# awentzonline/tartangan

Measured on AMD Instinct MI355X. Metric: images/sec (G+D step), higher is better.
Workload: dtype f32; 1 GPU; 128:3 SA-GAN cnn G+D step (R1 penalty, Adam x2, EMA), 128x128 RGB, batch 64/GPU, global batch 64; trainer=cnn, gan_config=128:3, global_batch=64, parallelism=dp1, hip_graphs=True

## Files before the change

include/tartangan_amd.h:

```cpp
#ifndef TARTANGAN_AMD_H
#define TARTANGAN_AMD_H

#include <stddef.h>
#include <stdint.h>

#ifdef __cplusplus
extern "C" {
#endif

#define TG_OK 0
#define TG_EINVAL (-1)
#define TG_EUNSUPPORTED (-2)
#define TG_EWORKSPACE (-3)

int tg_version(void);
const char* tg_arch(void);

int tg_conv2d_fwd(const float* x, const float* w, const float* bias ,
                  const float* residual ,
                  float* y, int B, int Cin, int Cout, int H, int W, int ks, void* stream);
int tg_conv2d_fwd_up2res(const float* x, const float* w, const float* bias , const float* residual_lo,
                         float* y, int B, int Cin, int Cout, int H, int W, void* stream);
int tg_upconv3x3_weights(const float* w, float* wp, int Cout, int Cin, void* stream);
int tg_upconv3x3_fwd(const float* a, const float* wp, const float* bias , const float* residual ,
                     float* y, int B, int Cin, int Cout, int H, int W, void* stream);
int tg_upconv3x3_weights_t(const float* w, float* w4t, int Cout, int Cin, void* stream);
int tg_upconv3x3_weights_pair(const float* w, float* wp, float* w4t, int Cout, int Cin, void* stream);
int tg_upconv3x3_dgrad_supported(int B, int Cin, int Cout, int H, int W);
int tg_upconv3x3_dgrad(const float* gy, const float* w4t, float* ga, int B, int Cin, int Cout, int H, int W, void* stream);
int tg_poolconv3x3_weights(const float* w, float* w4, float* wp, int Cout, int Cin, void* stream);
int tg_poolconv3x3_supported(int B, int Cin, int Cout, int H, int W);
int tg_poolconv3x3_fwd(const float* x, const float* w4, const float* bias , const float* residual ,
                       float* y, int B, int Cin, int Cout, int H, int W, void* stream);
int tg_poolconv3x3_dgrad(const float* gy, const float* wp, float* gx, int B, int Cin, int Cout, int H, int W, void* stream);
size_t tg_poolconv3x3_wgrad_workspace(int B, int Cin, int Cout, int H, int W);
int tg_poolconv3x3_wgrad(const float* x , const float* gy , float* gw, float* workspace,
                         size_t workspace_bytes, int B, int Cin, int Cout, int H, int W, int accumulate, float* gbias ,
                         void* stream);
size_t tg_upconv3x3_wgrad_workspace(int B, int Cin, int Cout, int H, int W);
int tg_upconv3x3_wgrad(const float* a , const float* gy , float* gw, float* workspace,
                       size_t workspace_bytes, int B, int Cin, int Cout, int H, int W, int accumulate, float* gbias ,
                       void* stream);
int tg_conv2d_dgrad(const float* gy, const float* w, float* gx,
                    int B, int Cin, int Cout, int H, int W, int ks, void* stream);
size_t tg_conv2d_wgrad_workspace(int B, int Cin, int Cout, int H, int W, int ks);
int tg_conv2d_wgrad(const float* x, const float* gy, float* gw, float* gbias ,
                    float* workspace, size_t workspace_bytes,
                    int B, int Cin, int Cout, int H, int W, int ks, int accumulate, void* stream);
int tg_conv1x1_multi_supported(int c0, int c1, int c2, int B, int Cin, int H, int W);
int tg_conv1x1_multi_fwd(const float* x, const float* w, float* y0, float* y1, float* y2, int c0, int c1, int c2,
                         int B, int Cin, int H, int W, void* stream);
int tg_conv1x1_multi_dgrad(const float* gy0, const float* gy1, const float* gy2, const float* w, float* gx,
                           int c0, int c1, int c2, int B, int Cin, int H, int W, void* stream);
size_t tg_conv1x1_multi_wgrad_workspace(int c0, int c1, int c2, int B, int Cin, int H, int W);
int tg_conv1x1_multi_wgrad(const float* x, const float* gy0, const float* gy1, const float* gy2, float* gw,
                           float* workspace, size_t workspace_bytes, int c0, int c1, int c2, int B, int Cin, int H, int W,
                           int accumulate , void* stream);
typedef int64_t tg_host_i64;
#define TG_WGRAD_ITEM_FIELDS 10
int tg_conv2d_wgrad_partials(const float* x, const float* gy, float* workspace, size_t workspace_bytes,
                             int B, int Cin, int Cout, int H, int W, int ks, int want_bias, void* stream);
int tg_conv2d_wgrad_reduce_batch(const tg_host_i64* items , int n_items, void* stream);
#define TG_FORM_ITEM_FIELDS 5
int tg_poolconv3x3_weights_batch(const tg_host_i64* items , int n_items, void* stream);
int tg_rgb_compose_fwd(const float* w1, const float* b1, const float* w3, float* wc, int Cout, int C, int Cimg, void* stream);
int tg_rgb_compose_bwd(const float* gwc, const float* w1, const float* b1, const float* w3, float* gw1, float* gb1, float* gw3, int Cout,
                       int C, int Cimg, int accumulate, void* stream);
int tg_poolconv3x3_wgrad_partials(const float* x, const float* gy, float* workspace, size_t workspace_bytes, int B, int Cin, int Cout,
                                  int H, int W, int want_bias, void* stream);
int tg_upconv3x3_wgrad_partials(const float* a, const float* gy, float* workspace, size_t workspace_bytes, int B, int Cin, int Cout,
                                int H, int W, int want_bias, void* stream);
int tg_s2_wgrad_reduce_batch(const tg_host_i64* items , int n_items, void* stream);
int tg_channel_sum(const float* x, float* out, float* workspace, int B, int C, int HW, int accumulate,
                   void* stream);
int tg_channel_bcast(const float* v, float* out, int B, int C, int HW, void* stream);

int tg_gemm(const float* A, const float* Bm, float* C, const float* bias_n ,
            int M, int N, int K, int lda, int ldb, int ldc, int transA, int transB,
            int batch, int64_t strideA, int64_t strideB, int64_t strideC, float beta, void* stream);

size_t tg_bn_workspace(int B, int C, int HW);
int tg_bn_train_stats(const float* x, float* mean, float* invstd,
                      float* running_mean , float* running_var ,
                      int64_t* num_batches_tracked ,
                      float momentum, float eps, float* workspace, int B, int C, int HW, int replicate, void* stream);
int tg_bn_train_fwd(const float* x, float* mean, float* invstd,
                    float* running_mean , float* running_var ,
                    int64_t* num_batches_tracked , const float* gamma, const float* beta,
                    float slope, float momentum, float eps, float* z, float* workspace,
                    int B, int C, int HW, int replicate, void* stream);
int tg_bn_eval_stats(const float* running_mean, const float* running_var, float* mean, float* invstd,
                     float eps, int C, void* stream);
int tg_bn_act_fwd(const float* x, const float* mean, const float* invstd, const float* gamma,
                  const float* beta, float slope, float* z, int B, int C, int HW, void* stream);
int tg_bn_act_bwd(const float* gz, const float* x, const float* mean, const float* invstd,
                  const float* gamma, const float* beta, float slope, int training,
                  float* gx , float* ggamma, float* gbeta, float* workspace,
                  int B, int C, int HW, int accumulate ,
                  const float* gx_add ,
                  void* stream);
int tg_bn_train_fwd_groups(const float* x, float* mean, float* invstd,
                           float* running_mean , float* running_var ,
                           int64_t* num_batches_tracked , const float* gamma, const float* beta,
                           float slope, float momentum, float eps, float* z, float* workspace,
                           int groups, int B, int C, int HW, int replicate, void* stream);
int tg_bn_act_bwd_groups(const float* gz, const float* x, const float* mean, const float* invstd,
                         const float* gamma, const float* beta, float slope, int training,
                         float* gx , float* ggamma, float* gbeta, float* workspace,
                         int groups, int B, int C, int HW, int accumulate,
                         const float* gx_add , int add_groups, void* stream);
int tg_bn_act_dbwd(const float* v, const float* vgamma , const float* vbeta ,
                   const float* gz, const float* x, const float* mean, const float* invstd,
                   const float* gamma, const float* beta, float slope,
                   float* adj_gz, float* adj_x, float* adj_gamma, float* workspace,
                   int B, int C, int HW, int accumulate , void* stream);

int tg_bn_sync_stats_local(const float* x, double* sums , float* workspace, int B, int C, int HW,
                           void* stream);
int tg_bn_sync_stats_finish(const double* sums , int world, float* mean, float* invstd,
                            float* running_mean , float* running_var ,
                            int64_t* num_batches_tracked , float momentum, float eps,
                            int64_t count_global, int replicate, int C, void* stream);
int tg_bn_sync_bwd_local(const float* gz, const float* x, const float* mean, const float* invstd,
                         const float* gamma, const float* beta, float slope, double* sums ,
                         float* workspace, int B, int C, int HW, void* stream);
int tg_bn_sync_bwd_finish(const float* gz, const float* x, const float* mean, const float* invstd,
                          const float* gamma, const float* beta, float slope,
                          const double* local_sums , const double* global_sums ,
                          int64_t count_global, float* gx , float* ggamma, float* gbeta,
                          float* workspace, int B, int C, int HW, int accumulate,
                          const float* gx_add , void* stream);
int tg_bn_sync_dbwd_local(const float* v, const float* gz, const float* x, const float* mean,
                          const float* invstd, const float* gamma, const float* beta, float slope,
                          double* sums , float* workspace, int B, int C, int HW, void* stream);
int tg_bn_sync_dbwd_finish(const float* v, const float* gz, const float* x, const float* mean,
                           const float* invstd, const float* gamma, const float* beta, float slope,
                           const double* global_sums , int64_t count_global, int world,
                           float* adj_gz, float* adj_x, float* adj_gamma, float* workspace,
                           int B, int C, int HW, int accumulate , void* stream);

int tg_up2x(const float* x, float* y, float alpha, int BC, int H, int W, void* stream);
int tg_pool2(const float* x, const float* residual ,
             float* y, float alpha, int BC, int H, int W, void* stream);
int tg_bilinear_half_fwd(const float* x, float* y, int BC, int H, int W, void* stream);
int tg_bilinear_half_bwd(const float* gy, const float* residual , float* gx,
// ... 149 lines not shown
```

tartangan_amd/csrc/conv.hip:

```cpp
#include <cstdlib>
#include <type_traits>
#include <utility>

#include "common.h"

namespace {

typedef float f32x16 __attribute__((ext_vector_type(16)));
typedef float f32x4 __attribute__((ext_vector_type(4)));

constexpr int CT_THREADS = 256;

template <int TH_, int TW_, int NI_>
struct Geo {
  static constexpr int TH = TH_, TW = TW_, NI = NI_, NPIX = TH_ * TW_ * NI_;
  static_assert(NPIX == 256 || NPIX == 64, "a pixel tile is 256 pixels (waves split pixels) or 64 (waves split K)");
  static constexpr int PPW = (NPIX == 64) ? 64 : NPIX / 4;
  static_assert(TW_ % 4 == 0, "rows are staged as float4");
};
using G4 = Geo<4, 4, 16>;
using G8 = Geo<8, 8, 4>;
using G16 = Geo<16, 16, 1>;
using GX = Geo<8, 32, 1>;
using G4k = Geo<4, 4, 4>;
// ... 1088 lines not shown
      if ((i + 1) * CT_THREADS <= PCHP || i * CT_THREADS + wave * 64 < PCHP) dma16(rx, buf + (i * CT_THREADS + wave * 64) * 4, off);
    }
#pragma unroll
    for (int i = 0; i < NVG; ++i) {
      const int e = i * CT_THREADS + threadIdx.x;
      const int co = e / WGD_GYQ, q = e % WGD_GYQ;
      const int p = 4 * q;
      const int img = p / (G::TH * G::TW), rem = p % (G::TH * G::TW);
      const int hh = tc.h0 + rem / G::TW, ww = tc.w0 + rem % G::TW;
      const bool ok = (e < GCH) && (q < 64) && (co0 + co < s.Cout) && (tc.b0 + img < s.B) && (hh < s.H) && (ww < s.W);
      const uint32_t off = ok ? (__umul24(__umul24(img, s.Cout) + co, HW) + __umul24(hh, s.W) + ww) << 2 : DMA_OOB;
      if ((i + 1) * CT_THREADS <= GCHP || i * CT_THREADS + wave * 64 < GCHP) dma16(rg, buf + PBUF + (i * CT_THREADS + wave * 64) * 4, off);
    }
  };
  auto compute = [&](const float* buf) {
    const float* pl = buf;
    const float* gl = buf + PBUF;
    if (s.prio) __builtin_amdgcn_s_setprio(0);
#pragma unroll
    for (int g = 0; g < 16; ++g) {
      constexpr int PPI = G::TH * G::TW;
      const int pg = 4 * g;
      const int goff = ((pg / PPI) * P::PH + (pg % PPI) / G::TW) * P::PWS + (pg % G::TW);
      float a[MTW], b[NT];
#pragma unroll
      for (int m = 0; m < MTW; ++m) a[m] = gl[lane_a + m * 16 * WG_GYS + 4 * g];
#pragma unroll
      for (int n = 0; n < NT; ++n) b[n] = pl[colbase[n] + lane_b + goff];
#pragma unroll
      for (int m = 0; m < MTW; ++m) bsum[m] += a[m];
#pragma unroll
      for (int m = 0; m < MTW; ++m)
#pragma unroll
        for (int n = 0; n < NT; ++n) acc[m][n] = __builtin_amdgcn_mfma_f32_16x16x4f32(a[m], b[n], acc[m][n], 0, 0, 0);
    }
    if (s.prio) __builtin_amdgcn_s_setprio(3);
  };

  for (int t = split; t < ntiles; t += S) {
    __syncthreads();
    issue(t, lds);
    asm volatile("s_waitcnt vmcnt(0)" ::: "memory");
    __syncthreads();
    compute(lds);
  }

  __syncthreads();
  float* red = lds;
#pragma unroll
  for (int m = 0; m < MTW; ++m)
#pragma unroll
    for (int n = 0; n < NT; ++n)
#pragma unroll
      for (int r = 0; r < 4; ++r) red[(((wave * MTW + m) * NT + n) * 4 + r) * 64 + lane] = acc[m][n][r];
  constexpr int PER_WAVE = MTW * NT * 4 * 64;
  float* bred = lds + 4 * PER_WAVE;
  if (do_bias) {
#pragma unroll
    for (int m = 0; m < MTW; ++m) {
      float v = bsum[m];
      v += __shfl_xor(v, 16, 64);
      v += __shfl_xor(v, 32, 64);
      if (h == 0) bred[wave * CT + m * 16 + j] = v;
    }
  }
  __syncthreads();
  for (int e = threadIdx.x; e < PER_WAVE; e += CT_THREADS) {
    const float v = (red[e] + red[PER_WAVE + e]) + (red[2 * PER_WAVE + e] + red[3 * PER_WAVE + e]);
    const int l = e & 63, q = e >> 6;
    const int r = q & 3, n = (q >> 2) % NT, m = (q >> 2) / NT;
    const int col = n * 16 + (l & 15);
    const int co = co0 + m * 16 + (l >> 4) * 4 + r;
    const int ci = ci0 + col / KK, tap = col % KK;
    if (col < NCOL && co < s.Cout && ci < s.Cin)
      part[(((int64_t)split * s.Cout + co) * s.Cin + ci) * KK + tap] = v;
  }
  if (do_bias && threadIdx.x < CT && co0 + (int)threadIdx.x < s.Cout) {
    const int c = threadIdx.x;
    bias_part[(int64_t)split * s.Cout + co0 + c] = (bred[c] + bred[CT + c]) + (bred[2 * CT + c] + bred[3 * CT + c]);
  }
}

template <int MT, int NT>
__global__ void __launch_bounds__(256)
conv1x1_wgrad_stream_kernel(const float* __restrict__ x, ChanSegs gys, float* __restrict__ part,
                            float* __restrict__ bias_part , int Cin, int Cout, int HW, int64_t groups, int S) {
  __shared__ float red[4 * MT * NT * 4 * 64 + 4 * 16 * MT];
  const int lane = threadIdx.x & 63, wave = threadIdx.x >> 6, j = lane & 15, h = lane >> 4;
  const int co0 = blockIdx.y * 16 * MT, ci0 = blockIdx.z * 16 * NT, split = blockIdx.x;
  const int64_t g_begin = groups * split / S, g_end = groups * (split + 1) / S;
  const int64_t n = g_end - g_begin;
  const int64_t w_begin = g_begin + n * wave / 4, w_end = g_begin + n * (wave + 1) / 4;
  const int gpp = HW >> 4;
  int64_t arow[MT], brow[NT], aimg[MT];
  const float* abase[MT];
#pragma unroll
  for (int m = 0; m < MT; ++m) {
    const int co = min(co0 + 16 * m + j, Cout - 1), k = gys.find(co);
    abase[m] = gys.p[k];
    aimg[m] = (int64_t)gys.width(k) * HW;
    arow[m] = (int64_t)(co - gys.start[k]) * HW + 4 * h;
  }
#pragma unroll
  for (int t = 0; t < NT; ++t) brow[t] = (int64_t)min(ci0 + 16 * t + j, Cin - 1) * HW + 4 * h;
  f32x4 acc[MT][NT];
#pragma unroll
  for (int m = 0; m < MT; ++m)
#pragma unroll
    for (int t = 0; t < NT; ++t) acc[m][t] = f32x4{0.f, 0.f, 0.f, 0.f};
  float bsum[MT];
#pragma unroll
  for (int m = 0; m < MT; ++m) bsum[m] = 0.f;
  constexpr int U = 4;
  for (int64_t g0 = w_begin; g0 < w_end; g0 += U) {
    float4 ga[U][MT], xb[U][NT];
#pragma unroll
    for (int u = 0; u < U; ++u) {
      const int64_t g = g0 + u;
      const bool ok = g < w_end;
      const int64_t b = ok ? g / gpp : 0;
      const int64_t p = ok ? (g - b * gpp) * 16 : 0;
#pragma unroll
      for (int m = 0; m < MT; ++m)
        ga[u][m] = ok ? *reinterpret_cast<const float4*>(abase[m] + b * aimg[m] + arow[m] + p) : make_float4(0.f, 0.f, 0.f, 0.f);
#pragma unroll
      for (int t = 0; t < NT; ++t)
        xb[u][t] = ok ? *reinterpret_cast<const float4*>(x + b * Cin * HW + brow[t] + p) : make_float4(0.f, 0.f, 0.f, 0.f);
    }
#pragma unroll
    for (int u = 0; u < U; ++u) {
#pragma unroll
      for (int m = 0; m < MT; ++m) bsum[m] += (ga[u][m].x + ga[u][m].y) + (ga[u][m].z + ga[u][m].w);
#pragma unroll
      for (int m = 0; m < MT; ++m) {
        const float av[4] = {ga[u][m].x, ga[u][m].y, ga[u][m].z, ga[u][m].w};
#pragma unroll
        for (int t = 0; t < NT; ++t) {
          const float bv[4] = {xb[u][t].x, xb[u][t].y, xb[u][t].z, xb[u][t].w};
#pragma unroll
          for (int r = 0; r < 4; ++r) acc[m][t] = __builtin_amdgcn_mfma_f32_16x16x4f32(av[r], bv[r], acc[m][t], 0, 0, 0);
        }
      }
    }
  }
  constexpr int PER_WAVE = MT * NT * 4 * 64;
#pragma unroll
  for (int m = 0; m < MT; ++m)
#pragma unroll
    for (int t = 0; t < NT; ++t)
#pragma unroll
      for (int i = 0; i < 4; ++i) red[wave * PER_WAVE + ((m * NT + t) * 4 + i) * 64 + lane] = acc[m][t][i];
  float* bred = red + 4 * PER_WAVE;
  const bool do_bias = bias_part != nullptr && blockIdx.z == 0;
  if (do_bias) {
#pragma unroll
    for (int m = 0; m < MT; ++m) {
      float v = bsum[m];
      v += __shfl_xor(v, 16, 64);
      v += __shfl_xor(v, 32, 64);
      if (h == 0) bred[wave * 16 * MT + 16 * m + j] = v;
    }
  }
  __syncthreads();
  for (int e = threadIdx.x; e < PER_WAVE; e += 256) {
    const float v = (red[e] + red[PER_WAVE + e]) + (red[2 * PER_WAVE + e] + red[3 * PER_WAVE + e]);
    const int l = e & 63, q = e >> 6;
    const int i = q & 3, t = (q >> 2) % NT, m = (q >> 2) / NT;
    const int co = co0 + 16 * m + 4 * (l >> 4) + i, ci = ci0 + 16 * t + (l & 15);
    if (co < Cout && ci < Cin) part[((int64_t)split * Cout + co) * Cin + ci] = v;
  }
  if (do_bias && threadIdx.x < 16 * MT && co0 + (int)threadIdx.x < Cout) {
    const int c = threadIdx.x;
    bias_part[(int64_t)split * Cout + co0 + c] = (bred[c] + bred[16 * MT + c]) + (bred[2 * 16 * MT + c] + bred[3 * 16 * MT + c]);
  }
}

static inline bool conv1x1_wgrad_stream_ok(const float* x, const float* gy, const Shape& s) {
  return (s.H * s.W) % 16 == 0 && tg_aligned16(x) && tg_aligned16(gy);
}
static int launch_conv1x1_wgrad_segs(const float* x, ChanSegs gy, float* part, float* bias_part, Shape s, int S, hipStream_t st) {
  const int HW = s.H * s.W;
  const int64_t groups = (int64_t)s.B * (HW / 16);
  const int mt = s.Cout > 16 ? 2 : 1, nt = s.Cin > 16 ? 2 : 1;
  dim3 grid(S, (s.Cout + 16 * mt - 1) / (16 * mt), (s.Cin + 16 * nt - 1) / (16 * nt));
  if (mt == 1 && nt == 1) conv1x1_wgrad_stream_kernel<1, 1><<<grid, 256, 0, st>>>(x, gy, part, bias_part, s.Cin, s.Cout, HW, groups, S);
  else if (mt == 1) conv1x1_wgrad_stream_kernel<1, 2><<<grid, 256, 0, st>>>(x, gy, part, bias_part, s.Cin, s.Cout, HW, groups, S);
  else if (nt == 1) conv1x1_wgrad_stream_kernel<2, 1><<<grid, 256, 0, st>>>(x, gy, part, bias_part, s.Cin, s.Cout, HW, groups, S);
  else conv1x1_wgrad_stream_kernel<2, 2><<<grid, 256, 0, st>>>(x, gy, part, bias_part, s.Cin, s.Cout, HW, groups, S);
  return tg_launch_status();
}
static int launch_conv1x1_wgrad_stream(const float* x, const float* gy, float* part, float* bias_part, Shape s, int S, hipStream_t st) {
  return launch_conv1x1_wgrad_segs(x, one_seg(gy, s.Cout), part, bias_part, s, S, st);
}

__device__ __forceinline__ void wgrad_reduce_block(int blk, const float* __restrict__ part, float* __restrict__ gw, int64_t E, int S,
                                                   const float* __restrict__ bias_part, float* __restrict__ gbias, int Cout,
                                                   int accumulate) {
  __shared__ float red[4][64];
  const int lane = threadIdx.x & 63, wave = threadIdx.x >> 6;
  const int eblocks = (int)((E + 63) / 64);
  const float* src = part;
  float* dst = gw;
  int64_t n = E, e = blk * 64ll + lane;
  if (blk >= eblocks) {
    src = bias_part; dst = gbias; n = Cout;
    e = (blk - eblocks) * 64ll + lane;
  }
  float a0 = 0.f, a1 = 0.f, a2 = 0.f, a3 = 0.f;
  if (e < n) {
    int sidx = wave;
    for (; sidx + 12 < S; sidx += 16) {
      a0 += src[(int64_t)sidx * n + e];
      a1 += src[(int64_t)(sidx + 4) * n + e];
      a2 += src[(int64_t)(sidx + 8) * n + e];
      a3 += src[(int64_t)(sidx + 12) * n + e];
    }
    for (; sidx < S; sidx += 4) a0 += src[(int64_t)sidx * n + e];
  }
  red[wave][lane] = (a0 + a1) + (a2 + a3);
  __syncthreads();
  if (wave == 0 && e < n) {
    const float r = (red[0][lane] + red[1][lane]) + (red[2][lane] + red[3][lane]);
    dst[e] = accumulate ? dst[e] + r : r;
  }
}

__global__ void __launch_bounds__(256) wgrad_reduce_kernel(const float* __restrict__ part, float* __restrict__ gw, int64_t E, int S,
                                                           const float* __restrict__ bias_part, float* __restrict__ gbias, int Cout,
                                                           int accumulate) {
  wgrad_reduce_block(blockIdx.x, part, gw, E, S, bias_part, gbias, Cout, accumulate);
}

constexpr int RB_MAX_ITEMS = 40;
struct ReduceItem {
  const float* part; float* gw; float* gbias;
  int64_t E;
  int S, Cout, accumulate, pad;
};
struct ReduceBatch {
  int n;
  int block_end[RB_MAX_ITEMS];
  ReduceItem item[RB_MAX_ITEMS];
};
__global__ void __launch_bounds__(256) wgrad_reduce_batch_kernel(ReduceBatch rb) {
  int i = 0;
  while (i + 1 < rb.n && (int)blockIdx.x >= rb.block_end[i]) ++i;
  const ReduceItem it = rb.item[i];
  const int blk = blockIdx.x - (i > 0 ? rb.block_end[i - 1] : 0);
  wgrad_reduce_block(blk, it.part, it.gw, it.E, it.S, it.gbias ? it.part + (int64_t)it.S * it.E : nullptr, it.gbias, it.Cout,
                     it.accumulate);
}

__global__ void __launch_bounds__(256) upconv_weights_kernel(const float* __restrict__ w, float* __restrict__ wp, int n ) {
  const int e = blockIdx.x * 256 + threadIdx.x;
  if (e >= n) return;
  float k[3][3];
#pragma unroll
  for (int i = 0; i < 9; ++i) k[i / 3][i % 3] = w[(int64_t)e * 9 + i];
#pragma unroll
  for (int dy = 0; dy < 2; ++dy)
#pragma unroll
    for (int dx = 0; dx < 2; ++dx) {
      float r[2][3];
#pragma unroll
      for (int c = 0; c < 3; ++c) {
        r[0][c] = dy == 0 ? k[0][c] : k[0][c] + k[1][c];
// ... 1739 lines not shown
                             int H, int W, int ks, int want_bias, void* stream) {
  TG_CHECK_PTR(x); TG_CHECK_PTR(gy); TG_CHECK_PTR(workspace);
  WgPlan p;
  return wgrad_partials(x, gy, workspace, workspace_bytes, B, Cin, Cout, H, W, ks, want_bias, tg_stream(stream), &p);
}

static inline bool qkv_ok(int c0, int c1, int c2, int B, int Cin, int H, int W) {
  const int C = c0 + c1 + c2;
  return c0 > 0 && c1 > 0 && c2 > 0 && C <= 64 && Cin <= 64 && (H * W) % 16 == 0 && check_shape(B, Cin, C, H, W, 1) == TG_OK;
}
int tg_conv1x1_multi_supported(int c0, int c1, int c2, int B, int Cin, int H, int W) { return qkv_ok(c0, c1, c2, B, Cin, H, W) ? 1 : 0; }

int tg_conv1x1_multi_fwd(const float* x, const float* w, float* y0, float* y1, float* y2, int c0, int c1, int c2, int B, int Cin,
                         int H, int W, void* stream) {
  TG_CHECK_PTR(x); TG_CHECK_PTR(w); TG_CHECK_PTR(y0); TG_CHECK_PTR(y1); TG_CHECK_PTR(y2);
  if (!qkv_ok(c0, c1, c2, B, Cin, H, W)) return TG_EUNSUPPORTED;
  if (!tg_aligned16(x) || !tg_aligned16(w) || !tg_aligned16(y0) || !tg_aligned16(y1) || !tg_aligned16(y2)) return TG_EUNSUPPORTED;
  Shape s{B, Cin, c0 + c1 + c2, H, W};
  return launch_conv1x1_segs(one_seg(x, Cin), w, nullptr, nullptr, three_segs(y0, y1, y2, c0, c1, c2), s, false, tg_stream(stream));
}

int tg_conv1x1_multi_dgrad(const float* gy0, const float* gy1, const float* gy2, const float* w, float* gx, int c0, int c1, int c2,
                           int B, int Cin, int H, int W, void* stream) {
  TG_CHECK_PTR(gy0); TG_CHECK_PTR(gy1); TG_CHECK_PTR(gy2); TG_CHECK_PTR(w); TG_CHECK_PTR(gx);
  if (!qkv_ok(c0, c1, c2, B, Cin, H, W)) return TG_EUNSUPPORTED;
  if (!tg_aligned16(gx) || !tg_aligned16(w) || !tg_aligned16(gy0) || !tg_aligned16(gy1) || !tg_aligned16(gy2)) return TG_EUNSUPPORTED;
  Shape s{B, c0 + c1 + c2, Cin, H, W};
  return launch_conv1x1_segs(three_segs(gy0, gy1, gy2, c0, c1, c2), w, nullptr, nullptr, one_seg(gx, Cin), s, true, tg_stream(stream));
}

size_t tg_conv1x1_multi_wgrad_workspace(int c0, int c1, int c2, int B, int Cin, int H, int W) {
  return tg_conv2d_wgrad_workspace(B, Cin, c0 + c1 + c2, H, W, 1);
}

int tg_conv1x1_multi_wgrad(const float* x, const float* gy0, const float* gy1, const float* gy2, float* gw, float* workspace,
                           size_t workspace_bytes, int c0, int c1, int c2, int B, int Cin, int H, int W, int accumulate, void* stream) {
  TG_CHECK_PTR(x); TG_CHECK_PTR(gy0); TG_CHECK_PTR(gy1); TG_CHECK_PTR(gy2); TG_CHECK_PTR(gw); TG_CHECK_PTR(workspace);
  if (!qkv_ok(c0, c1, c2, B, Cin, H, W)) return TG_EUNSUPPORTED;
  if (!tg_aligned16(x) || !tg_aligned16(gy0) || !tg_aligned16(gy1) || !tg_aligned16(gy2) || !tg_aligned16(gw) || !tg_aligned16(workspace))
    return TG_EUNSUPPORTED;
  const int C = c0 + c1 + c2;
  if (workspace_bytes < tg_conv2d_wgrad_workspace(B, Cin, C, H, W, 1)) return TG_EWORKSPACE;
  const WgPlan p = wgrad_plan(B, Cin, C, H, W, 1);
  Shape s{B, Cin, C, H, W};
  hipStream_t st = tg_stream(stream);
  if (int rc = launch_conv1x1_wgrad_segs(x, three_segs(gy0, gy1, gy2, c0, c1, c2), workspace, nullptr, s, p.S, st)) return rc;
  const int64_t E = (int64_t)C * Cin;
  wgrad_reduce_kernel<<<(int)((E + 63) / 64), 256, 0, st>>>(workspace, gw, E, p.S, nullptr, nullptr, C, accumulate);
  return tg_launch_status();
}

int tg_conv2d_wgrad_reduce_batch(const tg_host_i64* items, int n_items, void* stream) {
  if (n_items < 0) return TG_EINVAL;
  if (n_items == 0) return TG_OK;
  TG_CHECK_PTR(items);
  hipStream_t st = tg_stream(stream);
  for (int base = 0; base < n_items; base += RB_MAX_ITEMS) {
    ReduceBatch rb;
    rb.n = n_items - base < RB_MAX_ITEMS ? n_items - base : RB_MAX_ITEMS;
    int blocks = 0;
    for (int i = 0; i < rb.n; ++i) {
      const tg_host_i64* it = items + (size_t)(base + i) * TG_WGRAD_ITEM_FIELDS;
      const int B = (int)it[3], Cin = (int)it[4], Cout = (int)it[5], H = (int)it[6], W = (int)it[7], ks = (int)it[8];
      if (it[0] == 0 || it[1] == 0) return TG_EINVAL;
      if (int rc = check_shape(B, Cin, Cout, H, W, ks)) return rc;
      ReduceItem& r = rb.item[i];
      r.part = reinterpret_cast<const float*>(it[0]);
      r.gw = reinterpret_cast<float*>(it[1]);
      r.gbias = reinterpret_cast<float*>(it[2]);
      r.E = (int64_t)Cout * Cin * ks * ks;
      r.S = wgrad_plan(B, Cin, Cout, H, W, ks).S;
      r.Cout = Cout;
      r.accumulate = (int)it[9];
      r.pad = 0;
      blocks += (int)((r.E + 63) / 64) + (r.gbias ? (Cout + 63) / 64 : 0);
      rb.block_end[i] = blocks;
    }
    for (int i = rb.n; i < RB_MAX_ITEMS; ++i) rb.block_end[i] = blocks;
    wgrad_reduce_batch_kernel<<<blocks, 256, 0, st>>>(rb);
  }
  return tg_launch_status();
}

}
```

tartangan_amd/csrc/elementwise.hip:

```cpp
#include "common.h"

namespace {

constexpr int EW_BLOCK = 256;
constexpr int RED_BLOCK = 256;
constexpr int RED_MAX_BLOCKS = 1024;

struct OpAdd { __device__ float operator()(float a, float b) const { return a + b; } };
struct OpMul { __device__ float operator()(float a, float b) const { return a * b; } };
struct OpLreluBwd {
  float slope;
  __device__ float operator()(float g, float x) const { return x > 0.f ? g : g * slope; }
};
struct OpTanhBwd {
  __device__ float operator()(float g, float y) const { return g * (1.f - y * y); }
};
struct OpEluBwd {
  float negcoef, poscoef; int order;
  __device__ float operator()(float g, float x) const {
    if (x <= 0.f) return g * negcoef * expf(x);
    return order == 1 ? g * poscoef : 0.f;
  }
};
struct OpScaleAdd {
// ... 303 lines not shown
int tg_elu_bwd(const float* g, const float* x, float alpha, float scale, int order, float* out, int64_t n, void* stream) {
  if (order != 1 && order != 2) return TG_EINVAL;
  return launch_binary(g, x, out, n, stream, OpEluBwd{alpha * scale, scale, order});
}
int tg_copy_channels(const float* src, float* dst, int B, int Cs, int Cd, int HW, float fill, void* stream) {
  TG_CHECK_PTR(src); TG_CHECK_PTR(dst);
  TG_CHECK_POS(B); TG_CHECK_POS(Cs); TG_CHECK_POS(Cd); TG_CHECK_POS(HW);
  const int64_t planes_dst = (int64_t)B * Cd;
  if (HW % 4 == 0 && tg_aligned16(src) && tg_aligned16(dst))
    copy_channels_kernel<4><<<tg_ew_grid(planes_dst * (HW / 4), EW_BLOCK), EW_BLOCK, 0, tg_stream(stream)>>>(src, dst, planes_dst, Cs, Cd, HW, fill);
  else
    copy_channels_kernel<1><<<tg_ew_grid(planes_dst * HW, EW_BLOCK), EW_BLOCK, 0, tg_stream(stream)>>>(src, dst, planes_dst, Cs, Cd, HW, fill);
  return tg_launch_status();
}
int tg_fill(float* x, float value, int64_t n, void* stream) { return launch_unary<OpFill, false>(nullptr, x, n, stream, OpFill{value}); }

size_t tg_reduce_workspace(int64_t n) { (void)n; return (size_t)RED_MAX_BLOCKS * sizeof(double); }

int tg_dot(const float* a, const float* b, float alpha, float* out, float* workspace, int64_t n, int accumulate, void* stream) {
  TG_CHECK_PTR(b);
  return launch_reduce(a, b, (double)alpha, out, workspace, n, stream, RedDot{}, accumulate);
}
int tg_sumsq(const float* x, float alpha, float* out, float* workspace, int64_t n, void* stream) {
  return launch_reduce(x, nullptr, (double)alpha, out, workspace, n, stream, RedSumSq{});
}

int tg_bce_logits(const float* logits, const float* targets, float* loss, float* dlogits, float* workspace, int n, void* stream) {
  TG_CHECK_PTR(logits); TG_CHECK_PTR(targets); TG_CHECK_PTR(loss); TG_CHECK_PTR(dlogits); TG_CHECK_PTR(workspace);
  TG_CHECK_POS(n);
  double* partial = reinterpret_cast<double*>(workspace);
  const int g = red_grid(n);
  bce_stage1<<<g, RED_BLOCK, 0, tg_stream(stream)>>>(logits, targets, dlogits, partial, n, Finish{g == 1 ? loss : nullptr, 1.0 / (double)n, 0});
  if (g > 1) reduce_stage2<<<1, RED_BLOCK, 0, tg_stream(stream)>>>(partial, g, 1.0 / (double)n, loss);
  return tg_launch_status();
}

int tg_info_code_loss(const float* codes, const float* z, const float* base, float w, float* out, float* dcodes, float* workspace,
                      int B, int C, int K, int ldz, void* stream) {
  TG_CHECK_PTR(codes); TG_CHECK_PTR(z); TG_CHECK_PTR(out); TG_CHECK_PTR(dcodes);
  TG_CHECK_POS(B);
  if (C < 0 || K < 0 || C + K == 0 || ldz < C + K) return TG_EINVAL;
  (void)workspace;
  info_code_loss_kernel<<<1, INFO_BLOCK, 0, tg_stream(stream)>>>(codes, z, base, w, out, dcodes, B, C, K, ldz);
  return tg_launch_status();
}

int tg_iqn_loss_groups(const float* preds, const float* target, const float* taus, float k, float* loss, float* dpreds,
                       float* workspace, int Q, int B, int groups, void* stream) {
  TG_CHECK_PTR(preds); TG_CHECK_PTR(target); TG_CHECK_PTR(taus); TG_CHECK_PTR(loss); TG_CHECK_PTR(dpreds); TG_CHECK_PTR(workspace);
  TG_CHECK_POS(Q); TG_CHECK_POS(B); TG_CHECK_POS(groups);
  double* partial = reinterpret_cast<double*>(workspace);
  const int g = red_grid((int64_t)Q * B * groups);
  iqn_loss_stage1<<<g, RED_BLOCK, 0, tg_stream(stream)>>>(preds, target, taus, k, dpreds, partial, Q, B, groups,
                                                          Finish{g == 1 ? loss : nullptr, 1.0 / (double)B, 0});
  if (g > 1) reduce_stage2<<<1, RED_BLOCK, 0, tg_stream(stream)>>>(partial, g, 1.0 / (double)B, loss);
  return tg_launch_status();
}
int tg_iqn_loss(const float* preds, const float* target, const float* taus, float k, float* loss, float* dpreds,
                float* workspace, int Q, int B, void* stream) {
  return tg_iqn_loss_groups(preds, target, taus, k, loss, dpreds, workspace, Q, B, 1, stream);
}

int tg_iqn_cos_embed(const float* taus, const float* range, float* out, int n, int dims, void* stream) {
  TG_CHECK_PTR(taus); TG_CHECK_PTR(range); TG_CHECK_PTR(out);
  TG_CHECK_POS(n); TG_CHECK_POS(dims);
  iqn_cos_embed_kernel<<<tg_ew_grid((int64_t)n * dims, EW_BLOCK), EW_BLOCK, 0, tg_stream(stream)>>>(taus, range, out, n, dims);
  return tg_launch_status();
}

int tg_adam_step(float* p, const float* g, float* m, float* v, const float* hyper, float eps, int64_t n, void* stream) {
  TG_CHECK_PTR(p); TG_CHECK_PTR(g); TG_CHECK_PTR(m); TG_CHECK_PTR(v); TG_CHECK_PTR(hyper);
  if (n <= 0) return TG_EINVAL;
  adam_kernel<<<tg_ew_grid(n, EW_BLOCK), EW_BLOCK, 0, tg_stream(stream)>>>(p, g, m, v, hyper, eps, n);
  return tg_launch_status();
}

int tg_ema(float* t, const float* p, float lr, int64_t n, void* stream) {
  TG_CHECK_PTR(t); TG_CHECK_PTR(p);
  if (n <= 0) return TG_EINVAL;
  ema_kernel<<<tg_ew_grid(n, EW_BLOCK), EW_BLOCK, 0, tg_stream(stream)>>>(t, p, lr, n);
  return tg_launch_status();
}

int tg_version(void) { return 107; }
const char* tg_arch(void) { return "gfx950"; }

}
```

tartangan_amd/functional.py:

```python
import contextlib
import weakref

import torch
from torch.autograd.function import once_differentiable

from . import backend as _be


class Function(torch.autograd.Function):
    handles_none_grads = False

    def __init_subclass__(cls, **kw):
        super().__init_subclass__(**kw)
        fwd, bwd = cls.__dict__.get('forward'), cls.__dict__.get('backward')
        if isinstance(fwd, staticmethod) and isinstance(bwd, staticmethod):
            cls.forward = staticmethod(_wrap_forward(cls, fwd.__func__))
            cls.backward = staticmethod(_wrap_backward(cls, bwd.__func__))


def _wrap_forward(cls, fwd):
    def forward(ctx, *args):
        out = fwd(ctx, *args)
        ctx.set_materialize_grads(False)
        ctx._n_inputs = len(args)
# ... 351 lines not shown

def per_half(fn, x, *args, **kw):
    r = fn(x.r, *args, **kw)
    f = fn(x.f, *args, **kw)
    return Pair(r, f)


class _ConvFwd(Function):

    @staticmethod
    def forward(ctx, x, w, bias, residual=None, residual_up=False):
        x, w = x.contiguous(), w.contiguous()
        B, Cin, H, W = x.shape
        Cout, ks = w.shape[0], w.shape[2]
        y = x.new_empty(B, Cout, H, W)
        if residual is not None:
            residual = residual.contiguous()
        if residual_up:
            if residual is None or ks != 3 or tuple(residual.shape) != (B, Cout, H // 2, W // 2) or H % 2 or W % 2:
                raise RuntimeError('residual_up needs a (B, Cout, H/2, W/2) residual on a 3x3 convolution of an even plane')
            K().conv2d_fwd_up2res(x, w, bias, residual, y, B, Cin, Cout, H, W)
        else:
            K().conv2d_fwd(x, w, bias, residual, y, B, Cin, Cout, H, W, ks)
        ctx.save_for_backward(x, w, bias)
        ctx.has_residual = residual is not None
        ctx.residual_up = residual_up
        ctx.data_input = is_data(x)
        return y

    @staticmethod
    def backward(ctx, gy):
        x, w, bias = ctx.saved_tensors
        gy = gy.contiguous()
        gx = gw = gb = None
        need_w = ctx.needs_input_grad[1] and _param_grads_wanted()
        need_b = bias is not None and ctx.needs_input_grad[2] and _param_grads_wanted()
        if ctx.needs_input_grad[0] and not _skip_input_grad(ctx):
            gx = _ConvDgrad.apply(gy, w)
        sink_w, sink_b = _grad_sink(w), _grad_sink(bias)
        if need_w and sink_w is not None and (not need_b or sink_b is not None):
            _conv_wgrad_into(x, gy, sink_w, sink_b if need_b else None, w.shape[2], accumulate=1)
        else:
            if need_w:
                gw = _ConvWgrad.apply(x, gy, w.shape[2])
            if need_b:
                gb = _ChannelSum.apply(gy)
        gres = None
        if ctx.has_residual and ctx.needs_input_grad[3]:
            gres = _Pool2.apply(gy, 1.0) if ctx.residual_up else gy
        return gx, gw, gb, gres, None


class _ConvDgrad(Function):
    @staticmethod
    def forward(ctx, gy, w):
        gy, w = gy.contiguous(), w.contiguous()
        B, Cout, H, W = gy.shape
        Cin, ks = w.shape[1], w.shape[2]
        gx = gy.new_empty(B, Cin, H, W)
        K().conv2d_dgrad(gy, w, gx, B, Cin, Cout, H, W, ks)
        ctx.save_for_backward(gy, w)
        return gx

    @staticmethod
    def backward(ctx, v):
        gy, w = ctx.saved_tensors
        v = v.contiguous()
        a_gy = a_w = None
        if ctx.needs_input_grad[0]:
            a_gy = _ConvFwd.apply(v, w, None, None)
        if ctx.needs_input_grad[1]:
            sink = _grad_sink(w) if _param_grads_wanted() else None
            if sink is not None:
                _conv_wgrad_into(v, gy, sink, None, w.shape[2], accumulate=1)
            else:
                a_w = _ConvWgrad.apply(v, gy, w.shape[2])
        return a_gy, a_w


class _DeferredWgrad:
    active = False
    items = []
    s2_items = []
    keep = []


@contextlib.contextmanager
def deferred_wgrad():
    outer = _DeferredWgrad.active
    _DeferredWgrad.active = True
    try:
        with grads_into_buckets():
            yield
    finally:
        _DeferredWgrad.active = outer
        if not outer:
            flush_wgrad()


class _WgradStream:
    import os as _os
    enabled = _os.environ.get('TG_WGRAD_STREAM', '0') == '1'
    stream = None
    used = False


@contextlib.contextmanager
def _beside_backward(*operands):
    st = _WgradStream
    if not (st.enabled and _DeferredWgrad.active and operands[0].is_cuda):
        yield
        return
    if st.stream is None:
        st.stream = torch.cuda.Stream()
    st.stream.wait_stream(torch.cuda.current_stream())
    _DeferredWgrad.keep.append(operands)
    st.used = True
    with torch.cuda.stream(st.stream):
        yield


def flush_wgrad():
    st = _DeferredWgrad
    if _WgradStream.used:
        torch.cuda.current_stream().wait_stream(_WgradStream.stream)
        _WgradStream.used = False
        if not st.items and not st.s2_items:
            st.keep = []
    if st.items or st.s2_items:
        items, st.items = st.items, []
        s2_items, st.s2_items = st.s2_items, []
        try:
            def in_rounds(table):
                rounds, seen = [], {}
                for row in table:
                    k = seen.get(row[1], 0)
                    seen[row[1]] = k + 1
                    if k == len(rounds):
                        rounds.append([])
                    rounds[k].append(row)
                return rounds
            for rows in in_rounds(items):
                K().conv2d_wgrad_reduce_batch(torch.tensor(rows, dtype=torch.int64), len(rows))
            for rows in in_rounds(s2_items):
                K().s2_wgrad_reduce_batch(torch.tensor(rows, dtype=torch.int64), len(rows))
        finally:
            st.keep = []


def _conv_wgrad_into(x, gy, gw, gbias, ks, accumulate):
    B, Cin, H, W = x.shape
    Cout = gy.shape[1]
    nbytes = K().conv2d_wgrad_workspace(B, Cin, Cout, H, W, ks)
    if accumulate and _DeferredWgrad.active:
        ws = x.new_empty(nbytes // 4 + 4)
        with _beside_backward(x, gy, ws):
            K().conv2d_wgrad_partials(x, gy, ws, ws.numel() * 4, B, Cin, Cout, H, W, ks, int(gbias is not None))
        _DeferredWgrad.items.append([ws.data_ptr(), gw.data_ptr(), gbias.data_ptr() if gbias is not None else 0,
                                     B, Cin, Cout, H, W, ks, 1])
        _DeferredWgrad.keep.append((ws, gw, gbias))
        return
    ws = _ws(x, nbytes)
    K().conv2d_wgrad(x, gy, gw, gbias, ws, ws.numel() * 4, B, Cin, Cout, H, W, ks, accumulate)


def _s2_wgrad_into(mode, lo_or_x, gy, gw, gbias, B, Cin, Cout, H, W):
    name = 'poolconv3x3' if mode == 0 else 'upconv3x3'
    nbytes = getattr(K(), name + '_wgrad_workspace')(B, Cin, Cout, H, W)
    if _DeferredWgrad.active:
        ws = gy.new_empty(nbytes // 4 + 4)
        with _beside_backward(lo_or_x, gy, ws):
            getattr(K(), name + '_wgrad_partials')(lo_or_x, gy, ws, ws.numel() * 4, B, Cin, Cout, H, W, int(gbias is not None))
        _DeferredWgrad.s2_items.append([ws.data_ptr(), gw.data_ptr(), gbias.data_ptr() if gbias is not None else 0,
                                        B, Cin, Cout, H, W, mode, 1])
        _DeferredWgrad.keep.append((ws, gw, gbias))
        return
    ws = _ws(gy, nbytes)
    with _beside_backward(lo_or_x, gy, ws):
        getattr(K(), name + '_wgrad')(lo_or_x, gy, gw, ws, ws.numel() * 4, B, Cin, Cout, H, W, 1, gbias)


class _ConvWgrad(Function):
    @staticmethod
    def forward(ctx, x, gy, ks):
        x, gy = x.contiguous(), gy.contiguous()
        gw = x.new_empty(gy.shape[1], x.shape[1], ks, ks)
        _conv_wgrad_into(x, gy, gw, None, ks, accumulate=0)
        ctx.save_for_backward(x, gy)
        return gw

    @staticmethod
    def backward(ctx, vw):
        x, gy = ctx.saved_tensors
        vw = vw.contiguous()
        a_x = a_gy = None
        if ctx.needs_input_grad[0]:
            a_x = _ConvDgrad.apply(gy, vw)
        if ctx.needs_input_grad[1]:
            a_gy = _ConvFwd.apply(x, vw, None, None)
        return a_x, a_gy, None


class _ChannelSum(Function):
    @staticmethod
    def forward(ctx, x):
        x = x.contiguous()
        B, C = x.shape[0], x.shape[1]
        hw = x[0, 0].numel()
        out = x.new_empty(C)
        K().channel_sum(x, out, _ws(x, K().bn_workspace(B, C, hw)), B, C, hw, 0)
        ctx.shape = x.shape
        return out

    @staticmethod
    def backward(ctx, v):
        return _ChannelBcast.apply(v, ctx.shape)


class _ChannelBcast(Function):
    @staticmethod
    def forward(ctx, v, shape):
        v = v.contiguous()
        out = v.new_empty(shape)
        hw = 1
        for s in shape[2:]:
            hw *= s
        K().channel_bcast(v, out, shape[0], shape[1], hw)
        return out

    @staticmethod
    def backward(ctx, g):
        return _ChannelSum.apply(g), None


def conv2d(x, weight, bias=None, residual=None, residual_up=False):
    if _is_pair(x):
        return pair_apply(_ConvFwd, x, weight, bias, residual, residual_up)
    return _ConvFwd.apply(x, weight, bias, residual, residual_up)


# ... 171 lines not shown

def skipgram_step(U, V, words, contexts, negatives, lr, padding_idx=None, loss_out=None):
    vocab, E = U.shape
    for name, idx in (('words', words), ('contexts', contexts), ('negatives', negatives)):
        _check_indexes('skipgram_step ' + name, idx, vocab)
    if not (U.is_contiguous() and V.is_contiguous()) or U.shape != V.shape:
        raise RuntimeError('skipgram_step: two contiguous tables of one shape')
    dev = U.device
    words, contexts, negatives = (t.to(device=dev, dtype=torch.int64).contiguous() for t in (words, contexts, negatives))
    B, C2 = contexts.shape
    if tuple(words.shape) != (B,) or tuple(negatives.shape) != (B, C2):
        raise RuntimeError('skipgram_step: words (B), contexts (B, C2), negatives (B, C2)')
    if loss_out is None:
        loss_out = torch.empty((), dtype=U.dtype, device=dev)
    ws = _ws(U, K().skipgram_workspace(B, C2, E))
    with torch.no_grad():
        K().skipgram_step(U, V, words, contexts, negatives, float(lr), -1 if padding_idx is None else int(padding_idx), loss_out, ws,
                          ws.numel() * 4, B, C2, E, vocab)
    return loss_out


class _ComposeRGB(Function):

    @staticmethod
    def forward(ctx, w1, b1, w3):
        w1, b1, w3 = w1.contiguous(), b1.contiguous(), w3.contiguous()
        Cout, C = w3.shape[:2]
        Cimg = w1.shape[1]
        wc = w3.new_empty(Cout, Cimg + 1, 3, 3)
        K().rgb_compose_fwd(w1, b1, w3, wc, Cout, C, Cimg)
        ctx.save_for_backward(w1, b1, w3)
        return wc

    @staticmethod
    @once_differentiable
    def backward(ctx, gwc):
        w1, b1, w3 = ctx.saved_tensors
        if not _param_grads_wanted() or not any(ctx.needs_input_grad):
            return None, None, None
        Cout, C = w3.shape[:2]
        Cimg = w1.shape[1]
        sinks = [_grad_sink(p) for p in (w1, b1, w3)]
        if all(ctx.needs_input_grad) and all(sk is not None for sk in sinks):
            K().rgb_compose_bwd(gwc.contiguous(), w1, b1, w3, sinks[0], sinks[1], sinks[2], Cout, C, Cimg, 1)
            return None, None, None
        g1, gb, g3 = torch.empty_like(w1), torch.empty_like(b1), torch.empty_like(w3)
        K().rgb_compose_bwd(gwc.contiguous(), w1, b1, w3, g1, gb, g3, Cout, C, Cimg, 0)
        need = ctx.needs_input_grad
        return (g1 if need[0] else None), (gb if need[1] else None), (g3 if need[2] else None)


def compose_rgb_filter(w1, b1, w3):
    return _ComposeRGB.apply(w1, b1, w3)


def _adjacent(ts):
    first = ts[0]
    if first is None:
        return None
    cols = first[0].numel()
    off = first.storage_offset()
    for t in ts:
        if (t is None or not t.is_contiguous() or t[0].numel() != cols or t.dtype != first.dtype
                or t.untyped_storage().data_ptr() != first.untyped_storage().data_ptr() or t.storage_offset() != off):
            return None
        off += t.numel()
    return first.as_strided((sum(t.shape[0] for t in ts), cols), (cols, 1), first.storage_offset())


def _stacked(ws):
    view = _adjacent(ws)
    return view if view is not None else torch.cat([w.reshape(w.shape[0], -1) for w in ws])


def _qkv_wgrad(x, gys, ws, need):
    if not any(need) or not _param_grads_wanted():
        return [None, None, None]
    sinks = [_grad_sink(w) for w in ws]
    cat = _adjacent(sinks) if all(need) and all(sk is not None for sk in sinks) else None
    if cat is None:
        return [_ConvWgrad.apply(x, g, 1) if n else None for g, n in zip(gys, need)]
    B, Cin, H, W = x.shape
    cs = [w.shape[0] for w in ws]
    nbytes = K().conv1x1_multi_wgrad_workspace(*cs, B, Cin, H, W)
    wsb = _ws(x, nbytes)
    K().conv1x1_multi_wgrad(x, gys[0], gys[1], gys[2], cat, wsb, wsb.numel() * 4, *cs, B, Cin, H, W, 1)
    return [None, None, None]


class _QKV(Function):

    @staticmethod
    def forward(ctx, x, wt, wp, wg):
        x = x.contiguous()
        B, Cin, H, W = x.shape
        cs = (wt.shape[0], wp.shape[0], wg.shape[0])
        ys = [x.new_empty(B, c, H, W) for c in cs]
        K().conv1x1_multi_fwd(x, _stacked((wt, wp, wg)), ys[0], ys[1], ys[2], *cs, B, Cin, H, W)
        ctx.save_for_backward(x, wt, wp, wg)
        ctx.data_input = is_data(x)
        return tuple(ys)

    @staticmethod
    def backward(ctx, gt, gp, gg):
        x, wt, wp, wg = ctx.saved_tensors
        gys = [g.contiguous() for g in (gt, gp, gg)]
        gx = None
        if ctx.needs_input_grad[0] and not _skip_input_grad(ctx):
            gx = _QKVDgrad.apply(gys[0], gys[1], gys[2], wt, wp, wg)
        gws = _qkv_wgrad(x, gys, (wt, wp, wg), ctx.needs_input_grad[1:4])
        return (gx, *gws)


class _QKVDgrad(Function):

    @staticmethod
    def forward(ctx, gt, gp, gg, wt, wp, wg):
        gys = [g.contiguous() for g in (gt, gp, gg)]
        B, _, H, W = gys[0].shape
        Cin = wt[0].numel()
        cs = (wt.shape[0], wp.shape[0], wg.shape[0])
        gx = gys[0].new_empty(B, Cin, H, W)
        K().conv1x1_multi_dgrad(gys[0], gys[1], gys[2], _stacked((wt, wp, wg)), gx, *cs, B, Cin, H, W)
        ctx.save_for_backward(gys[0], gys[1], gys[2], wt, wp, wg)
        return gx

    @staticmethod
    def backward(ctx, v):
        gt, gp, gg, wt, wp, wg = ctx.saved_tensors
        v = v.contiguous()
        a_g = [None, None, None]
        if any(ctx.needs_input_grad[:3]):
            a_g = list(_QKV.apply(v, wt, wp, wg))
        a_w = _qkv_wgrad(v, (gt, gp, gg), (wt, wp, wg), ctx.needs_input_grad[3:6])
        return (*a_g, *a_w)


def qkv_supported(x, w_theta, w_phi, w_g):
    B, Cin, H, W = x.shape
    cs = (w_theta.shape[0], w_phi.shape[0], w_g.shape[0])
    return all(bool(K().conv1x1_multi_supported(*cs, b, Cin, H, W)) for b in ((B, B // 2) if _is_pair(x) else (B,)))


def qkv_projections(x, w_theta, w_phi, w_g):
    if _is_pair(x):
        return pair_apply(_QKV, x, w_theta, w_phi, w_g)
    return _QKV.apply(x, w_theta, w_phi, w_g)


PAIR_SPECS[_QKV] = ('b---', 'h---', 'bbb')


class _UpConv3x3(Function):

    @staticmethod
    def forward(ctx, a, w, bias, residual=None):
        a, w = a.contiguous(), w.contiguous()
        B, Cin, H, W = a.shape
        Cout = w.shape[0]
        if w.shape[2:] != (3, 3):
            raise RuntimeError('upconv3x3 needs a 3x3 filter')
        wp = a.new_empty(4, Cout, Cin, 2, 2)
        ctx.w4t = None
        need = getattr(ctx, 'needs_input_grad', ())
        if need and need[0] and K().upconv3x3_dgrad_supported(B, Cin, Cout, H, W):
            ctx.w4t = a.new_empty(Cin, Cout, 4, 4)
# ... 2134 lines not shown
```

Before: 6996 images/s.

## Batch deferred 1x1 conv weight-grad partials into one grouped kernel launch

Adds a grouped kernel that processes a table of 1x1 conv wgrad partial jobs (single-output and fused QKV) in one launch, and queues these jobs during backward instead of launching one kernel per conv. The queued batch runs at flush time ahead of the existing reduce rounds. The goal is fewer launches and better GPU fill for small convs. In exchange, the partials no longer overlap with the rest of backward, and each job now gets its own workspace allocation.

```diff
diff --git a/include/tartangan_amd.h b/include/tartangan_amd.h
--- a/include/tartangan_amd.h
+++ b/include/tartangan_amd.h
@@ -61,6 +61,9 @@
 int tg_conv2d_wgrad_partials(const float* x, const float* gy, float* workspace, size_t workspace_bytes,
                              int B, int Cin, int Cout, int H, int W, int ks, int want_bias, void* stream);
 int tg_conv2d_wgrad_reduce_batch(const tg_host_i64* items , int n_items, void* stream);
+#define TG_WGRAD1X1_ITEM_FIELDS 15
+int tg_conv1x1_wgrad_batch_supported(int B, int Cin, int Cout, int H, int W);
+int tg_conv1x1_wgrad_partials_batch(const tg_host_i64* items , int n_items, void* stream);
 #define TG_FORM_ITEM_FIELDS 5
 int tg_poolconv3x3_weights_batch(const tg_host_i64* items , int n_items, void* stream);
 int tg_rgb_compose_fwd(const float* w1, const float* b1, const float* w3, float* wc, int Cout, int C, int Cimg, void* stream);
diff --git a/tartangan_amd/csrc/conv.hip b/tartangan_amd/csrc/conv.hip
--- a/tartangan_amd/csrc/conv.hip
+++ b/tartangan_amd/csrc/conv.hip
@@ -1194,12 +1194,12 @@
 }
 
 template <int MT, int NT>
-__global__ void __launch_bounds__(256)
-conv1x1_wgrad_stream_kernel(const float* __restrict__ x, ChanSegs gys, float* __restrict__ part,
-                            float* __restrict__ bias_part , int Cin, int Cout, int HW, int64_t groups, int S) {
-  __shared__ float red[4 * MT * NT * 4 * 64 + 4 * 16 * MT];
+__device__ __forceinline__ void
+conv1x1_wgrad_stream_body(float* red, const float* __restrict__ x, const ChanSegs& gys, float* __restrict__ part,
+                          float* __restrict__ bias_part , int Cin, int Cout, int HW, int64_t groups, int S,
+                          int split, int co_tile, int ci_tile) {
   const int lane = threadIdx.x & 63, wave = threadIdx.x >> 6, j = lane & 15, h = lane >> 4;
-  const int co0 = blockIdx.y * 16 * MT, ci0 = blockIdx.z * 16 * NT, split = blockIdx.x;
+  const int co0 = co_tile * 16 * MT, ci0 = ci_tile * 16 * NT;
   const int64_t g_begin = groups * split / S, g_end = groups * (split + 1) / S;
   const int64_t n = g_end - g_begin;
   const int64_t w_begin = g_begin + n * wave / 4, w_end = g_begin + n * (wave + 1) / 4;
@@ -1263,7 +1263,7 @@
 #pragma unroll
       for (int i = 0; i < 4; ++i) red[wave * PER_WAVE + ((m * NT + t) * 4 + i) * 64 + lane] = acc[m][t][i];
   float* bred = red + 4 * PER_WAVE;
-  const bool do_bias = bias_part != nullptr && blockIdx.z == 0;
+  const bool do_bias = bias_part != nullptr && ci_tile == 0;
   if (do_bias) {
 #pragma unroll
     for (int m = 0; m < MT; ++m) {
@@ -1287,13 +1287,59 @@
   }
 }
 
+template <int MT, int NT>
+__global__ void __launch_bounds__(256)
+conv1x1_wgrad_stream_kernel(const float* __restrict__ x, ChanSegs gys, float* __restrict__ part,
+                            float* __restrict__ bias_part , int Cin, int Cout, int HW, int64_t groups, int S) {
+  __shared__ float red[4 * MT * NT * 4 * 64 + 4 * 16 * MT];
+  conv1x1_wgrad_stream_body<MT, NT>(red, x, gys, part, bias_part, Cin, Cout, HW, groups, S, blockIdx.x, blockIdx.y, blockIdx.z);
+}
+
+constexpr int W1B_MAX_ITEMS = 40;
+struct Wgrad1x1Item {
+  const float* x;
+  ChanSegs gy;
+  float* part; float* bias_part;
+  int64_t groups;
+  int Cin, Cout, HW, S;
+};
+struct Wgrad1x1Batch {
+  int n;
+  int block_end[W1B_MAX_ITEMS];
+  Wgrad1x1Item item[W1B_MAX_ITEMS];
+};
+static_assert(sizeof(Wgrad1x1Batch) <= 4096, "the table travels in the kernel argument block");
+__host__ __device__ static inline int conv1x1_wgrad_mt(int Cout) { return Cout > 16 ? 2 : 1; }
+__host__ __device__ static inline int conv1x1_wgrad_nt(int Cin) { return Cin > 16 ? 2 : 1; }
+
+__global__ void __launch_bounds__(256) conv1x1_wgrad_grouped_kernel(Wgrad1x1Batch tb) {
+  __shared__ float red[4 * 2 * 2 * 4 * 64 + 4 * 16 * 2];
+  int i = 0;
+  while (i + 1 < tb.n && (int)blockIdx.x >= tb.block_end[i]) ++i;
+  const Wgrad1x1Item& it = tb.item[i];
+  int l = blockIdx.x - (i > 0 ? tb.block_end[i - 1] : 0);
+  const int mt = conv1x1_wgrad_mt(it.Cout), nt = conv1x1_wgrad_nt(it.Cin);
+  const int co_tiles = (it.Cout + 16 * mt - 1) / (16 * mt);
+  const int split = l % it.S;
+  l /= it.S;
+  const int co_tile = l % co_tiles, ci_tile = l / co_tiles;
+  if (mt == 1 && nt == 1)
+    conv1x1_wgrad_stream_body<1, 1>(red, it.x, it.gy, it.part, it.bias_part, it.Cin, it.Cout, it.HW, it.groups, it.S, split, co_tile, ci_tile);
+  else if (mt == 1)
+    conv1x1_wgrad_stream_body<1, 2>(red, it.x, it.gy, it.part, it.bias_part, it.Cin, it.Cout, it.HW, it.groups, it.S, split, co_tile, ci_tile);
+  else if (nt == 1)
+    conv1x1_wgrad_stream_body<2, 1>(red, it.x, it.gy, it.part, it.bias_part, it.Cin, it.Cout, it.HW, it.groups, it.S, split, co_tile, ci_tile);
+  else
+    conv1x1_wgrad_stream_body<2, 2>(red, it.x, it.gy, it.part, it.bias_part, it.Cin, it.Cout, it.HW, it.groups, it.S, split, co_tile, ci_tile);
+}
+
 static inline bool conv1x1_wgrad_stream_ok(const float* x, const float* gy, const Shape& s) {
   return (s.H * s.W) % 16 == 0 && tg_aligned16(x) && tg_aligned16(gy);
 }
 static int launch_conv1x1_wgrad_segs(const float* x, ChanSegs gy, float* part, float* bias_part, Shape s, int S, hipStream_t st) {
   const int HW = s.H * s.W;
   const int64_t groups = (int64_t)s.B * (HW / 16);
-  const int mt = s.Cout > 16 ? 2 : 1, nt = s.Cin > 16 ? 2 : 1;
+  const int mt = conv1x1_wgrad_mt(s.Cout), nt = conv1x1_wgrad_nt(s.Cin);
   dim3 grid(S, (s.Cout + 16 * mt - 1) / (16 * mt), (s.Cin + 16 * nt - 1) / (16 * nt));
   if (mt == 1 && nt == 1) conv1x1_wgrad_stream_kernel<1, 1><<<grid, 256, 0, st>>>(x, gy, part, bias_part, s.Cin, s.Cout, HW, groups, S);
   else if (mt == 1) conv1x1_wgrad_stream_kernel<1, 2><<<grid, 256, 0, st>>>(x, gy, part, bias_part, s.Cin, s.Cout, HW, groups, S);
@@ -3199,4 +3245,67 @@
   return tg_launch_status();
 }
 
-}
+static inline bool wgrad1x1_shape_ok(int B, int Cin, int Cout, int H, int W) {
+  return check_shape(B, Cin, Cout, H, W, 1) == TG_OK && ((int64_t)H * W) % 16 == 0;
+}
+int tg_conv1x1_wgrad_batch_supported(int B, int Cin, int Cout, int H, int W) { return wgrad1x1_shape_ok(B, Cin, Cout, H, W) ? 1 : 0; }
+
+static int wgrad1x1_check_row(const tg_host_i64* it) {
+  const int64_t c0 = it[6], c1 = it[7], c2 = it[8];
+  for (int f = 6; f <= 14; ++f)
+    if (it[f] < 0 || it[f] > INT32_MAX) return TG_EINVAL;
+  const int B = (int)it[9], Cin = (int)it[10], H = (int)it[11], W = (int)it[12], ks = (int)it[13];
+  if (it[0] == 0 || it[1] == 0 || it[4] == 0 || c0 <= 0 || c0 + c1 + c2 > INT32_MAX) return TG_EINVAL;
+  const bool one = c1 == 0 && c2 == 0 && it[2] == 0 && it[3] == 0, three = c1 > 0 && c2 > 0 && it[2] != 0 && it[3] != 0;
+  if (!one && !three) return TG_EINVAL;
+  const int Cout = (int)(c0 + c1 + c2);
+  if (int rc = check_shape(B, Cin, Cout, H, W, ks)) return rc;
+  if (ks != 1 || !wgrad1x1_shape_ok(B, Cin, Cout, H, W)) return TG_EUNSUPPORTED;
+  for (int f = 0; f <= 4; ++f)
+    if (it[f] & 15) return TG_EUNSUPPORTED;
+  if (it[5] < 0 || (uint64_t)it[5] < tg_conv2d_wgrad_workspace(B, Cin, Cout, H, W, 1)) return TG_EWORKSPACE;
+  return TG_OK;
+}
+
+int tg_conv1x1_wgrad_partials_batch(const tg_host_i64* items, int n_items, void* stream) {
+  if (n_items < 0) return TG_EINVAL;
+  if (n_items == 0) return TG_OK;
+  TG_CHECK_PTR(items);
+  for (int i = 0; i < n_items; ++i)
+    if (int rc = wgrad1x1_check_row(items + (size_t)i * TG_WGRAD1X1_ITEM_FIELDS)) return rc;
+  hipStream_t st = tg_stream(stream);
+  for (int base = 0; base < n_items;) {
+    Wgrad1x1Batch tb;
+    int64_t blocks = 0;
+    int n = 0;
+    for (; n < W1B_MAX_ITEMS && base + n < n_items; ++n) {
+      const tg_host_i64* it = items + (size_t)(base + n) * TG_WGRAD1X1_ITEM_FIELDS;
+      const int c0 = (int)it[6], c1 = (int)it[7], c2 = (int)it[8], Cout = c0 + c1 + c2;
+      const int B = (int)it[9], Cin = (int)it[10], H = (int)it[11], W = (int)it[12], HW = H * W;
+      const WgPlan p = wgrad_plan(B, Cin, Cout, H, W, 1);
+      const int mt = conv1x1_wgrad_mt(Cout), nt = conv1x1_wgrad_nt(Cin);
+      const int64_t wgs = (int64_t)p.S * ((Cout + 16 * mt - 1) / (16 * mt)) * ((Cin + 16 * nt - 1) / (16 * nt));
+      if (n > 0 && blocks + wgs > INT32_MAX) break;
+      if (wgs > INT32_MAX) return TG_EUNSUPPORTED;
+      Wgrad1x1Item& w = tb.item[n];
+      float* ws = reinterpret_cast<float*>(it[4]);
+      w.x = reinterpret_cast<const float*>(it[0]);
+      w.gy = c1 ? three_segs(reinterpret_cast<const float*>(it[1]), reinterpret_cast<const float*>(it[2]), reinterpret_cast<const float*>(it[3]), c0, c1, c2)
+                : one_seg(reinterpret_cast<const float*>(it[1]), Cout);
+      w.part = ws;
+      w.bias_part = it[14] ? ws + (size_t)p.S * Cout * Cin : nullptr;
+      w.groups = (int64_t)B * (HW / 16);
+      w.Cin = Cin; w.Cout = Cout; w.HW = HW; w.S = p.S;
+      blocks += wgs;
+      tb.block_end[n] = (int)blocks;
+    }
+    tb.n = n;
+    for (int i = n; i < W1B_MAX_ITEMS; ++i) { tb.block_end[i] = (int)blocks; tb.item[i] = tb.item[0]; }
+    conv1x1_wgrad_grouped_kernel<<<(unsigned)blocks, 256, 0, st>>>(tb);
+    if (int rc = tg_launch_status()) return rc;
+    base += n;
+  }
+  return TG_OK;
+}
+
+}
diff --git a/tartangan_amd/csrc/elementwise.hip b/tartangan_amd/csrc/elementwise.hip
--- a/tartangan_amd/csrc/elementwise.hip
+++ b/tartangan_amd/csrc/elementwise.hip
@@ -409,7 +409,7 @@
   return tg_launch_status();
 }
 
-int tg_version(void) { return 107; }
+int tg_version(void) { return 108; }
 const char* tg_arch(void) { return "gfx950"; }
 
 }
diff --git a/tartangan_amd/functional.py b/tartangan_amd/functional.py
--- a/tartangan_amd/functional.py
+++ b/tartangan_amd/functional.py
@@ -457,7 +457,36 @@
     active = False
     items = []
     s2_items = []
+    stage1 = []
     keep = []
+
+
+GROUPED_WGRAD_MAX_BYTES = None
+
+
+def _grouped_stage1_enabled():
+    return not _WgradStream.enabled and hasattr(K(), 'conv1x1_wgrad_partials_batch')
+
+
+def _grouped_stage1(x, gys, ws, cs, want_bias):
+    k = K()
+    if not _grouped_stage1_enabled():
+        return False
+    B, Cin, H, W = x.shape
+    ts = (x, *gys, ws)
+    if isinstance(k, _be.HipBackend) and not all(t.is_cuda for t in ts):
+        return False
+    if not all(t.is_contiguous() and t.dtype == torch.float32 and t.data_ptr() % 16 == 0 for t in ts):
+        return False
+    if not k.conv1x1_wgrad_batch_supported(B, Cin, sum(cs), H, W):
+        return False
+    if GROUPED_WGRAD_MAX_BYTES is not None and 4 * B * H * W * (Cin + sum(cs)) > GROUPED_WGRAD_MAX_BYTES:
+        return False
+    ptrs = [g.data_ptr() for g in gys] + [0] * (3 - len(gys))
+    widths = list(cs) + [0] * (3 - len(cs))
+    _DeferredWgrad.stage1.append([x.data_ptr(), *ptrs, ws.data_ptr(), ws.numel() * 4, *widths, B, Cin, H, W, 1, int(want_bias)])
+    _DeferredWgrad.keep.append(ts)
+    return True
 
 
 @contextlib.contextmanager
@@ -505,7 +534,10 @@
     if st.items or st.s2_items:
         items, st.items = st.items, []
         s2_items, st.s2_items = st.s2_items, []
+        stage1, st.stage1 = st.stage1, []
         try:
+            if stage1:
+                K().conv1x1_wgrad_partials_batch(torch.tensor(stage1, dtype=torch.int64), len(stage1))
             def in_rounds(table):
                 rounds, seen = [], {}
                 for row in table:
@@ -529,8 +561,9 @@
     nbytes = K().conv2d_wgrad_workspace(B, Cin, Cout, H, W, ks)
     if accumulate and _DeferredWgrad.active:
         ws = x.new_empty(nbytes // 4 + 4)
-        with _beside_backward(x, gy, ws):
-            K().conv2d_wgrad_partials(x, gy, ws, ws.numel() * 4, B, Cin, Cout, H, W, ks, int(gbias is not None))
+        if not (ks == 1 and _grouped_stage1(x, (gy,), ws, (Cout,), gbias is not None)):
+            with _beside_backward(x, gy, ws):
+                K().conv2d_wgrad_partials(x, gy, ws, ws.numel() * 4, B, Cin, Cout, H, W, ks, int(gbias is not None))
         _DeferredWgrad.items.append([ws.data_ptr(), gw.data_ptr(), gbias.data_ptr() if gbias is not None else 0,
                                      B, Cin, Cout, H, W, ks, 1])
         _DeferredWgrad.keep.append((ws, gw, gbias))
@@ -868,6 +901,13 @@
         return [_ConvWgrad.apply(x, g, 1) if n else None for g, n in zip(gys, need)]
     B, Cin, H, W = x.shape
     cs = [w.shape[0] for w in ws]
+    if _DeferredWgrad.active and _grouped_stage1_enabled():
+        C = sum(cs)
+        wsd = x.new_empty(K().conv2d_wgrad_workspace(B, Cin, C, H, W, 1) // 4 + 4)
+        if _grouped_stage1(x, tuple(gys), wsd, cs, False):
+            _DeferredWgrad.items.append([wsd.data_ptr(), cat.data_ptr(), 0, B, Cin, C, H, W, 1, 1])
+            _DeferredWgrad.keep.append((wsd, cat))
+            return [None, None, None]
     nbytes = K().conv1x1_multi_wgrad_workspace(*cs, B, Cin, H, W)
     wsb = _ws(x, nbytes)
     K().conv1x1_multi_wgrad(x, gys[0], gys[1], gys[2], cat, wsb, wsb.numel() * 4, *cs, B, Cin, H, W, 1)
```

New measurement: 7097 images/s (median of 6 runs). 1.4% higher.
